# gsneha26/SegAlign

Measured on AMD Instinct MI355X. Metric: Gbp query seeded+filtered+extended per sec, higher is better.
Workload: dtype int32

## Files before the change

segalign_amd/csrc/extend.hip:

```cpp
#include <atomic>
#include <cstdlib>

#include "kernels.h"
#include "kmer_dev.h"

namespace sa {

constexpr int EXT_THREADS = 256;
constexpr int NEG = -(1 << 26);
constexpr int DEAD = -(1 << 29);
constexpr uint64_t TERM_ALL = 0x4040404040404040ull;
constexpr uint32_t BIAS = SEQ_PAD;

__device__ __forceinline__ int f64_to_i32(double x) { return (int)x; }

enum : int { PH_RIGHT = 0, PH_LEFT = 1, PH_FIN = 2, PH_IDLE = 3 };

template <int CTRL, int ROW_MASK = 0xf, int BANK_MASK = 0xf>
__device__ __forceinline__ int dpp_mov(int old, int v) {
    return __builtin_amdgcn_update_dpp(old, v, CTRL, ROW_MASK, BANK_MASK, false);
}
__device__ __forceinline__ uint32_t wave_inclusive_sum(uint32_t v) {
    v += (uint32_t)dpp_mov<0x111>(0, (int)v);
    v += (uint32_t)dpp_mov<0x112>(0, (int)v);
// ... 557 lines not shown
                        }
                        const uint32_t rp = (td >> (4 * j)) & 15u;
                        const uint32_t addr = (rp << 2) | qaddr;
                        const s16x2 e = __builtin_bit_cast(s16x2, *reinterpret_cast<const uint32_t*>(reinterpret_cast<const char*>(s_pk) + addr));
                        const s16x2 Tb = T.yy;
                        T = __builtin_elementwise_add_sat(Tb, e);
                        M = __builtin_elementwise_max(M, T);
                    }
                    m = max((int)M.x, (int)M.y);
                    alive = (m - (int)T.y) <= xdrop;
                }
            }
            walked += 64;
            if (!alive) {
                if (!left) {
                    bestR = m;
                    if (SRC == SRC_CAND && left_known) {
                        best = left_best;
                        phase = PH_FIN;
                    } else {
                        phase = PH_LEFT;
                        walked = 0;
                        T = (s16x2){0, 0};
                        M = (s16x2){0, 0};
                    }
                } else {
                    best = m;
                    phase = PH_FIN;
                }
            } else if (walked + (uint32_t)(64 - CTX_R_BASES) >= long_cap) {
                forward = true;
                phase = PH_FIN;
            }
        }

        const unsigned long long fin = __ballot(phase == PH_FIN);
        const unsigned long long live = __ballot(phase < PH_FIN);
        if (fin != 0ull && (__popcll(fin) >= fin_batch || live == 0ull)) {
            bool cand = false;
            if (phase == PH_FIN && has_hit) cand = forward || bound_passes(a, bestR + best);
            {
                CandRec cr;
                cr.ref_loc = ref_loc; cr.query_loc = query_loc; cr.hidx = hidx;
                stage_append(stage, n_stage, cand, cr, a.cand_list, a.cand_count, a.cand_cap_recs, lane, lane_lt);
            }
            if (a.audit_list) {
                uint2 ar;
                ar.x = ref_loc; ar.y = query_loc;
                wave_append(phase == PH_FIN && has_hit && !cand, ar, a.audit_list, a.audit_count, a.audit_cap, lane, lane_lt);
            }
            unsigned long long need = fin;
            bool got = false;
            Hit mine = {0u, 0u};
            uint32_t mine_idx = 0, mine_known = 0, mine_tm = 0, mine_flags = 3;
            while (need != 0ull) {
                const int avail = buf_cnt - consumed;
                if (avail <= 0) {
                    if (nxt_cnt == 0) break;
                    buf = nxt;
                    buf_idx = nxt_idx;
                    buf_known = nxt_known; buf_tm = nxt_tm; buf_flags = nxt_flags;
                    buf_cnt = nxt_cnt;
                    cur_buf = nxt_buf;
                    consumed = 0;
                    nxt_buf += G;
                    nxt_cnt = buf_count(nxt_buf);
                    nxt = fetch(nxt_buf, nxt_cnt);
                    nxt_idx = f_idx;
                    nxt_known = f_known; nxt_tm = f_tm; nxt_flags = f_flags;
                    continue;
                }
                const int rank = __popcll(need & lane_lt);
                const bool take = ((need >> lane) & 1ull) && rank < avail;
                const int src = (consumed + rank) & 63;
                const uint32_t hr = (uint32_t)__shfl((int)buf.ref_loc, src, 64);
                const uint32_t hq = (uint32_t)__shfl((int)buf.query_loc, src, 64);
                const uint32_t hi = SRC == SRC_CAND ? (uint32_t)__shfl((int)buf_idx, src, 64) : (uint32_t)(cur_buf << 6) + (uint32_t)src;
                uint32_t hk = 0, ht = 0, hf = 3;
                if (SRC == SRC_CAND) {
                    hk = (uint32_t)__shfl((int)buf_known, src, 64);
                    ht = (uint32_t)__shfl((int)buf_tm, src, 64);
                    hf = (uint32_t)__shfl((int)buf_flags, src, 64);
                }
                if (take) {
                    mine.ref_loc = hr;
                    mine.query_loc = hq;
                    mine_idx = hi;
                    mine_known = hk; mine_tm = ht; mine_flags = hf;
                    got = true;
                }
                consumed += min(__popcll(need), avail);
                need &= ~__ballot(take);
            }
            if (phase == PH_FIN) {
                forward = false;
                if (got) {
                    has_hit = true;
                    ref_loc = mine.ref_loc;
                    query_loc = mine.query_loc;
                    hidx = mine_idx;
                    bestR = 0;
                    best = 0;
                    bool skip = false;
                    if (a.rm) skip = !(ref_loc >= a.rm_win_start && ref_loc <= a.rm_win_end);
                    left_known = false;
                    if (skip || ref_loc > a.ref_len || query_loc > a.query_len) {
                        phase = PH_FIN;
                    } else if (SRC == SRC_CAND && mine_flags == 0u) {
                        bestR = (int)mine_known;
                        best = (int)mine_tm;
                        phase = PH_FIN;
                    } else if (SRC == SRC_CAND && mine_flags == 2u) {
                        bestR = (int)mine_known;
                        phase = PH_LEFT;
                        walked = (uint32_t)CTX_L_BASES + a.left_skip;
                        const short t16 = (short)(mine_tm & 0xFFFFu), m16 = (short)(mine_tm >> 16);
                        T = (s16x2){t16, t16};
                        M = (s16x2){m16, m16};
                    } else {
                        phase = PH_RIGHT;
                        walked = 0;
                        T = (s16x2){0, 0};
                        M = (s16x2){0, 0};
                        if (SRC == SRC_CAND && mine_flags == 1u) {
                            left_known = true;
                            left_best = (int)mine_known;
                            if (a.l2_right_state) {
                                walked = (uint32_t)CTX_R_BASES;
                                const short t16 = (short)(mine_tm & 0xFFFFu), m16 = (short)(mine_tm >> 16);
                                T = (s16x2){t16, t16};
                                M = (s16x2){m16, m16};
                            }
                        }
                    }
                } else {
                    has_hit = false;
                    phase = PH_IDLE;
                }
            }
        }
        if (__ballot(phase != PH_IDLE) == 0ull) break;
    }
    stage_flush(stage, n_stage, a.cand_list, a.cand_count, a.cand_cap_recs, lane);
}

constexpr int CTX_THREADS = 1024;
constexpr int CTX_THREADS_MAX = 1024;
constexpr int CTX_STAGE_FLUSH = 32;
constexpr int CTX_STAGE_CAP = CTX_STAGE_FLUSH - 1 + 64 + 1;
constexpr int CLS_TAB = 4096;
constexpr int CLS_TAIL = 256;
constexpr int CLS_LDS_DWORDS = CLS_TAB + CLS_TAIL;
constexpr bool CLS_TRACK_DROP = true;

__device__ __forceinline__ void cls_table_init(uint32_t* __restrict__ s_cls, const int* cls, int nthreads) {
    const int c0 = cls[0], c1 = cls[1], c2 = cls[2], c3 = cls[3];
    for (int i = threadIdx.x; i < CLS_TAB + CLS_TAIL; i += nthreads) {
        const int nb = i < CLS_TAB ? 6 : 4;
        const int f = i < CLS_TAB ? i : i - CLS_TAB;
        int sum = 0, mx = 0;
        for (int k = 0; k < nb; k++) {
            const int x = (f >> (2 * k)) & 3;
            sum += x == 0 ? c0 : x == 1 ? c1 : x == 2 ? c2 : c3;
            mx = max(mx, sum);
        }
        s_cls[i] = ((uint32_t)sum << 16) | ((uint32_t)(sum - mx) & 0xFFFFu);
    }
}

template <int O>
__device__ __forceinline__ uint32_t cls_field_addr(uint32_t w0, uint32_t w1) {
    constexpr uint32_t MASK = 0x3FFCu;
    if (O + 12 <= 32) return O >= 2 ? ((w0 >> (O - 2)) & MASK) : ((w0 << (2 - O)) & MASK);
    return __builtin_amdgcn_alignbit(w1, w0, (uint32_t)(O - 2)) & MASK;
}

__device__ __forceinline__ uint32_t mul24(uint32_t x, uint32_t s_uniform) {
    uint32_t r;
    asm("v_mul_u32_u24 %0, %1, %2" : "=v"(r) : "s"(s_uniform), "v"(x));
    return r;
}

__device__ __forceinline__ void cls_step(const uint32_t* __restrict__ s_tab, uint32_t addr, uint32_t& P, uint32_t& W) {
    const uint32_t e = *reinterpret_cast<const uint32_t*>(reinterpret_cast<const char*>(s_tab) + addr);
    asm("v_pk_add_i16 %0, %1, %2 op_sel:[0,1] op_sel_hi:[1,1]" : "=v"(P) : "v"(P), "v"(e));
    asm("v_min_i16_sdwa %0, %0, %1 dst_sel:WORD_0 dst_unused:UNUSED_PRESERVE src0_sel:WORD_0 src1_sel:WORD_0" : "+v"(P) : "v"(e));
    if (CLS_TRACK_DROP) {
        typedef short s16x2 __attribute__((ext_vector_type(2)));
        W = __builtin_bit_cast(uint32_t, __builtin_elementwise_min(__builtin_bit_cast(s16x2, W), __builtin_bit_cast(s16x2, P)));
    }
}

__device__ __forceinline__ uint32_t cls_seed_state(const ExtendArgs& a) {
    const int cmax = max(max(a.cls[0], a.cls[1]), max(a.cls[2], a.cls[3]));
    return (uint32_t)((int)a.left_skip * max(cmax, 0)) << 16;
}

template <bool ONE_COPY>
__global__ __launch_bounds__(CTX_THREADS_MAX, 8) void extend_filter_cls_kernel(ExtendArgs a) {
    __shared__ __attribute__((aligned(16))) uint32_t s_cls[CLS_LDS_DWORDS];
    extern __shared__ L2Rec s_l2_dyn[];
    cls_table_init(s_cls, a.cls, (int)blockDim.x);
    __syncthreads();
    const uint32_t* __restrict__ s_tail = s_cls + CLS_TAB;
    L2Rec* stage = s_l2_dyn + (threadIdx.x >> 6) * CTX_STAGE_CAP;
    int n_stage = 0;
    const int lane = threadIdx.x & 63;
    const unsigned long long lane_lt = (1ull << lane) - 1ull;
    const int xdrop = a.xdrop;
    const uint4* __restrict__ ctx = reinterpret_cast<const uint4*>(a.td_ctx);
    const uint32_t seed_state = cls_seed_state(a);

    const uint64_t num_buf = (a.num_hits + 63) >> 6;
    const uint64_t n_chunks = (a.num_hits + TD_CHUNK_HITS - 1) / TD_CHUNK_HITS;
    const uint64_t W = (uint64_t)gridDim.x * (blockDim.x >> 6);
    const uint64_t wid = (uint64_t)__builtin_amdgcn_readfirstlane((int)(blockIdx.x * (blockDim.x >> 6) + (threadIdx.x >> 6)));
    const uint64_t c_lo = (wid * n_chunks) / W, c_hi = ((wid + 1) * n_chunks) / W;
    const uint64_t b_lo = c_lo * (TD_CHUNK_HITS / 64);
    const uint64_t b_hi = min(c_hi * (TD_CHUNK_HITS / 64), num_buf);
    if (b_lo >= b_hi) return;
    const uint32_t my_sub = (uint32_t)wid & (uint32_t)(L2_NSUB - 1);
    L2Rec* __restrict__ my_list = a.l2_list + (size_t)my_sub * a.l2_cap;
    uint32_t* __restrict__ my_count = a.l2_count + my_sub * L2_CNT_STRIDE;
    typedef const uint64_t __attribute__((address_space(4))) * HeadPtr;
    HeadPtr head = (HeadPtr)a.td_bits;
    const uint32_t stride16 = (uint32_t)(a.q2_stride >> 4) & 0xFFFFFFu;
    uint32_t cbefore;
    auto locate = [&](uint64_t B) -> uint32_t {
        const uint64_t Bs = B >> 1;
        const uint32_t idx = __builtin_amdgcn_mbcnt_hi((uint32_t)(Bs >> 32), __builtin_amdgcn_mbcnt_lo((uint32_t)Bs, cbefore - 1u + (uint32_t)(B & 1ull)));
        cbefore += (uint32_t)__builtin_popcountll(B);
        return idx;
    };
    struct Stage {
        uint4 c0, tl;
        uint32_t q[7];
        uint32_t query_loc;
    };
    auto merge_q = [&](Stage& S, uint32_t qr0, uint32_t qr1, uint32_t qr2, uint32_t qr3, uint32_t ql0, uint32_t ql1, uint32_t ql2, uint32_t ql3) {
        S.q[0] = qr0; S.q[1] = qr1; S.q[2] = qr2;
        S.q[3] = (qr3 & 0xFFFu) | (ql0 << 12);
        S.q[4] = __builtin_amdgcn_alignbit(ql1, ql0, 20);
        S.q[5] = __builtin_amdgcn_alignbit(ql2, ql1, 20);
        S.q[6] = __builtin_amdgcn_alignbit(ql3, ql2, 20);
    };
    uint64_t w0, w1, w2;
    TdRec hnext;
    auto advance_map = [&](uint64_t b_req) {
        hnext = a.td_rec[locate(w0)];
        w0 = w1;
        w1 = w2;
        w2 = head[b_req + 4];
    };
    auto request = [&](uint64_t b, Stage& S) {
        const uint64_t entry = hnext.off + (uint64_t)((uint32_t)(b << 6) + (uint32_t)lane - hnext.prefix);
        S.c0 = ctx[2 * entry];
        S.tl = ctx[2 * entry + 1];
        const uint32_t query_loc = hnext.qpos + a.seed_size;
        S.query_loc = query_loc;
        const uint32_t lp = a.query_len - query_loc + a.left_skip;
        if (ONE_COPY) {
            uint4 t;
            uint32_t t4;
            const uint8_t* rpp = a.q2_own + ((query_loc >> 4) << 2);
            __builtin_memcpy(&t, __builtin_assume_aligned(rpp, 4), 16);
            __builtin_memcpy(&t4, __builtin_assume_aligned(rpp + 16, 4), 4);
            const uint32_t sr = (query_loc & 15u) << 1;
            uint4 u;
            uint32_t u4;
            const uint8_t* lpp = a.q2_other + ((lp >> 4) << 2);
            __builtin_memcpy(&u, __builtin_assume_aligned(lpp, 4), 16);
            __builtin_memcpy(&u4, __builtin_assume_aligned(lpp + 16, 4), 4);
            const uint32_t sl = (lp & 15u) << 1;
            merge_q(S, __builtin_amdgcn_alignbit(t.y, t.x, sr), __builtin_amdgcn_alignbit(t.z, t.y, sr), __builtin_amdgcn_alignbit(t.w, t.z, sr),
                    __builtin_amdgcn_alignbit(t4, t.w, sr), __builtin_amdgcn_alignbit(u.y, u.x, sl), __builtin_amdgcn_alignbit(u.z, u.y, sl),
                    __builtin_amdgcn_alignbit(u.w, u.z, sl), __builtin_amdgcn_alignbit(u4, u.w, sl));
        } else {
            const uint32_t po = (mul24(query_loc & 15u, stride16) << 4) + ((query_loc >> 4) << 2);
            uint4 t, u;
            __builtin_memcpy(&t, __builtin_assume_aligned(a.q2_own + po, 4), 16);
            const uint32_t qo = (mul24(lp & 15u, stride16) << 4) + ((lp >> 4) << 2);
            __builtin_memcpy(&u, __builtin_assume_aligned(a.q2_other + qo, 4), 16);
            merge_q(S, t.x, t.y, t.z, t.w, u.x, u.y, u.z, u.w);
        }
    };
    auto score = [&](uint64_t b, const Stage& S) {
        const bool valid = (b << 6) + (uint64_t)lane < a.num_hits;
        const uint32_t query_loc = S.query_loc;
        const uint32_t ref_loc = S.c0.x + a.seed_size;
        bool skip = !valid;
        if (a.rm) skip = skip || !(ref_loc >= a.rm_win_start && ref_loc <= a.rm_win_end);
        const uint32_t x0 = S.c0.y ^ S.q[0], x1 = S.c0.z ^ S.q[1], x2 = S.c0.w ^ S.q[2], x3 = S.tl.x ^ S.q[3], x4 = S.tl.y ^ S.q[4],
                       x5 = S.tl.z ^ S.q[5], x6 = S.tl.w ^ S.q[6];
        uint32_t P = 0, Wd = 0;
        cls_step(s_cls, cls_field_addr<0>(x0, x1), P, Wd);
        cls_step(s_cls, cls_field_addr<12>(x0, x1), P, Wd);
        cls_step(s_cls, cls_field_addr<24>(x0, x1), P, Wd);
        cls_step(s_cls, cls_field_addr<4>(x1, x2), P, Wd);
        cls_step(s_cls, cls_field_addr<16>(x1, x2), P, Wd);
        cls_step(s_cls, cls_field_addr<28>(x1, x2), P, Wd);
        cls_step(s_cls, cls_field_addr<8>(x2, x3), P, Wd);
        cls_step(s_cls, cls_field_addr<20>(x2, x3), P, Wd);
        cls_step(s_cls, cls_field_addr<0>(x3, x4), P, Wd);
        const bool r_alive = (int)(short)((CLS_TRACK_DROP ? Wd : P) & 0xFFFFu) >= -xdrop;
        const int bestR = ((int)P >> 16) - (int)(short)(P & 0xFFFFu);
        const uint32_t PR = P;
        P = seed_state; Wd = 0;
        cls_step(s_cls, cls_field_addr<12>(x3, x4), P, Wd);
        cls_step(s_cls, cls_field_addr<24>(x3, x4), P, Wd);
        cls_step(s_cls, cls_field_addr<4>(x4, x5), P, Wd);
        cls_step(s_cls, cls_field_addr<16>(x4, x5), P, Wd);
        cls_step(s_cls, cls_field_addr<28>(x4, x5), P, Wd);
        cls_step(s_cls, cls_field_addr<8>(x5, x6), P, Wd);
        cls_step(s_cls, cls_field_addr<20>(x5, x6), P, Wd);
        cls_step(s_cls, cls_field_addr<0>(x6, 0u), P, Wd);
        cls_step(s_cls, cls_field_addr<12>(x6, 0u), P, Wd);
        cls_step(s_tail, (x6 >> 22) & 0x3FCu, P, Wd);
        const bool l_alive = (int)(short)((CLS_TRACK_DROP ? Wd : P) & 0xFFFFu) >= -xdrop;
        const int bestL = ((int)P >> 16) - (int)(short)(P & 0xFFFFu);
        const bool fwd = !skip && (r_alive || l_alive || bound_passes(a, bestR + bestL));
        const unsigned long long fm = __ballot(fwd);
        if (fm) {
            L2Rec cr;
            cr.ref_loc = ref_loc;
            cr.query_loc = query_loc;
            cr.hidx = (uint32_t)(b << 6) + (uint32_t)lane;
            const uint32_t fl = (r_alive ? 1u : 0u) | (l_alive ? 2u : 0u);
            const uint32_t Ps = (fl == 1u && a.l2_right_state) ? PR : P;
            cr.state = (Ps & 0xFFFF0000u) | ((0u - Ps) & 0xFFFFu);
            cr.meta = (uint32_t)(r_alive ? bestL : bestR) | ((fl ? fl : 3u) << 16);
            const uint32_t rank = __builtin_amdgcn_mbcnt_hi((uint32_t)(fm >> 32), __builtin_amdgcn_mbcnt_lo((uint32_t)fm, 0u));
            if (fwd) stage[n_stage + (int)rank] = cr;
            n_stage += __popcll(fm);
            __builtin_amdgcn_wave_barrier();
            if (n_stage >= CTX_STAGE_FLUSH) {
                const int k = n_stage < 64 ? n_stage : 64;
                stage_flush(stage, k, my_list, my_count, a.l2_cap, lane);
                const int rest = n_stage - k;
                L2Rec tmp = cr;
                if (lane < rest) tmp = stage[k + lane];
                __builtin_amdgcn_wave_barrier();
                if (lane < rest) stage[lane] = tmp;
                __builtin_amdgcn_wave_barrier();
                n_stage = rest;
            }
        }
        if (a.audit_list) {
            uint2 ar;
            ar.x = ref_loc;
            ar.y = query_loc;
            wave_append(valid && !skip && !fwd, ar, a.audit_list, a.audit_count, a.audit_cap, lane, lane_lt);
        }
    };
    Stage SA, SB;
    {
        const uint64_t h0 = head[b_lo];
        w0 = head[b_lo + 1];
        w1 = head[b_lo + 2];
        w2 = head[b_lo + 3];
        cbefore = a.td_chunk[c_lo] + 1u - (uint32_t)(h0 & 1ull);
        hnext = a.td_rec[locate(h0)];
        request(b_lo, SA);
        advance_map(b_lo);
    }
    for (uint64_t b = b_lo; b < b_hi; b += 2) {
        request(b + 1, SB);
        advance_map(b + 1);
        score(b, SA);
        if (b + 1 >= b_hi) break;
        request(b + 2, SA);
        advance_map(b + 2);
        score(b + 1, SB);
    }
    stage_flush(stage, n_stage, my_list, my_count, a.l2_cap, lane);
}

__device__ __forceinline__ int rfl(int v) { return __builtin_amdgcn_readfirstlane(v); }

template <bool COUNT_EXAMINED, bool XDROP_NONNEG>
__device__ __forceinline__ void wave_extend_exact(const ExtendArgs& a, const int* __restrict__ s_tab,
                                                  const uint8_t* __restrict__ R8b, const uint8_t* __restrict__ Qb, int lane,
                                                  uint32_t ref_loc, uint32_t query_loc, int& bestR, int& bposR, int& bestL,
                                                  int& boffL, unsigned long long& examined) {
    const int xdrop = a.xdrop;
    bestR = 0; bposR = -1; bestL = 0; boffL = 0;
    bool skip = false;
    if (a.rm) skip = !(ref_loc >= a.rm_win_start && ref_loc <= a.rm_win_end);
    if (skip) bposR = 0;
    for (int side = skip ? 2 : 0; side < 2; side++) {
        const bool left = side == 1;
        const uint32_t lim = left ? min(ref_loc, query_loc)
                                  : ((ref_loc < a.ref_len && query_loc < a.query_len)
                                         ? min(a.ref_len - ref_loc, a.query_len - query_loc) : 0u);
        uint32_t k0 = left ? 1u : 0u;
        int score_in = 0, best_in = 0, bpos_in = left ? 0 : -1;
        for (;;) {
            const uint32_t k = k0 + 8u * (uint32_t)lane;
            const int64_t rem64 = left ? (int64_t)lim - (int64_t)k + 1 : (int64_t)lim - (int64_t)k;
            const int remaining = rem64 > 8 ? 8 : (rem64 < 0 ? 0 : (int)rem64);
            uint64_t x = 0;
            if (remaining > 0) {
                const uint32_t roff = left ? ref_loc + BIAS - k - 7u : ref_loc + BIAS + k;
                const uint32_t qoff = left ? query_loc + BIAS - k - 7u : query_loc + BIAS + k;
                x = load8u(R8b + roff) | load8u(Qb + qoff);
                if (left) x = __builtin_bswap64(x);
            }
            if (remaining < 8) x |= (remaining <= 0) ? TERM_ALL : (TERM_ALL << (8 * remaining));
            uint32_t run = 0;
            int mx = INT32_MIN, amx = 0;
            {
                const uint32_t xlo = (uint32_t)x, xhi = (uint32_t)(x >> 32);
#pragma unroll
                for (int j = 0; j < 8; j++) {
                    const uint32_t w = j < 4 ? xlo : xhi;
                    run += (uint32_t)s_tab[(w >> (8 * (j & 3))) & 0xffu];
                    const bool up = (int)run > mx;
                    amx = up ? j : amx;
                    mx = up ? (int)run : mx;
                }
            }
            const uint32_t inc = wave_inclusive_sum(run);
            const int base = (int)((uint32_t)score_in + inc - run);
            int mv = (int)((uint32_t)base + (uint32_t)mx), mp = (int)(k + (uint32_t)amx);
            wave_inclusive_max(mv, mp);
            int ev = dpp_mov<0x138>(INT32_MIN, mv);
            int ep = dpp_mov<0x138>(0, mp);
            if (best_in >= ev) { ev = best_in; ep = bpos_in; }
            int score = base, best = ev, bpos = ep;
            uint32_t ex_step = 0;
            chunk8_exact<COUNT_EXAMINED, XDROP_NONNEG>(s_tab, x, k, xdrop, score, best, bpos, ex_step);
            const unsigned long long dm = __ballot(score < (DEAD >> 1));
            if (dm) {
                const int f = __ffsll((long long)dm) - 1;
                best_in = __builtin_amdgcn_readlane(best, f);
                bpos_in = __builtin_amdgcn_readlane(bpos, f);
                if (COUNT_EXAMINED && lane <= f) examined += ex_step;
                break;
            }
            if (COUNT_EXAMINED) examined += ex_step;
            score_in = __builtin_amdgcn_readlane(score, 63);
            best_in = __builtin_amdgcn_readlane(best, 63);
            bpos_in = __builtin_amdgcn_readlane(bpos, 63);
            k0 += 512u;
        }
        if (!left) { bestR = best_in; bposR = bpos_in; }
        else { bestL = best_in; boffL = bpos_in; }
    }
}

struct ExactStage {
    HspRec* st_out;
    EntRec* st_ent;
    int n_out, n_ent;
};

__device__ __forceinline__ void wave_finalize(const ExtendArgs& a, ExactStage& st, int lane, uint32_t ref_loc, uint32_t query_loc,
                                              uint32_t seg, int bestR, int bposR, int bestL, int boffL) {
    const int total = bestR + bestL, extent = bposR + boffL;
    const int cls = classify(a, total);
    if (!cls) return;
    if (cls == 1) {
        if (lane == 0) st.st_out[st.n_out] = make_rec(a, ref_loc, query_loc, boffL, extent, total, seg);
        st.n_out++;
        __builtin_amdgcn_wave_barrier();
        if (st.n_out == 64) { stage_flush(st.st_out, 64, a.out, a.out_count, a.out_cap, lane); st.n_out = 0; __builtin_amdgcn_wave_barrier(); }
    } else {
        if (lane == 0) {
            EntRec er;
            er.ref_loc = ref_loc; er.query_loc = query_loc; er.bposR = bposR; er.boffL = boffL; er.total = total; er.seg = seg;
            st.st_ent[st.n_ent] = er;
        }
        st.n_ent++;
        __builtin_amdgcn_wave_barrier();
        if (st.n_ent == 64) { stage_flush(st.st_ent, 64, a.ent_list, a.ent_count, a.ent_cap_recs, lane); st.n_ent = 0; __builtin_amdgcn_wave_barrier(); }
    }
}

#define EXACT_KERNEL_PROLOGUE()                                                                            \
    __shared__ int s_tab[128];                                                                             \
    __shared__ HspRec s_out[EXT_THREADS / 64][64];                                                         \
    __shared__ EntRec s_ent[EXT_THREADS / 64][64];                                                         \
    if (threadIdx.x < 128) s_tab[threadIdx.x] = threadIdx.x < 64 ? a.sub_mat[threadIdx.x] : NEG;           \
    __syncthreads();                                                                                       \
    ExactStage st = {s_out[threadIdx.x >> 6], s_ent[threadIdx.x >> 6], 0, 0};                             \
    const int lane = threadIdx.x & 63;                                                                     \
    const uint8_t* __restrict__ R8b = a.ref8 - BIAS;                                                       \
    const uint8_t* __restrict__ Qb = a.query - BIAS;                                                       \
    const uint32_t n_cand = min(*a.cand_count, a.cand_cap_recs);                                           \
    const uint32_t G = gridDim.x * (EXT_THREADS / 64);                                                     \
    SEG_TABLE()                                                                                            \
    unsigned long long examined = 0;

#define EXACT_KERNEL_EPILOGUE()                                                                            \
    stage_flush(st.st_out, st.n_out, a.out, a.out_count, a.out_cap, lane);                                 \
    stage_flush(st.st_ent, st.n_ent, a.ent_list, a.ent_count, a.ent_cap_recs, lane);                       \
    if (COUNT_EXAMINED) {                                                                                  \
        unsigned long long v = examined;                                                                   \
        for (int off = 32; off > 0; off >>= 1) v += __shfl_down(v, off, 64);                               \
        if (lane == 0 && v) atomicAdd(a.examined, v);                                                      \
    }

template <bool COUNT_EXAMINED, bool XDROP_NONNEG>
__global__ __launch_bounds__(EXT_THREADS) void extend_exact_kernel(ExtendArgs a) {
    EXACT_KERNEL_PROLOGUE()
    if (a.chain_cap && n_cand <= a.chain_cap) return;
    for (uint32_t i = blockIdx.x * (EXT_THREADS / 64) + (threadIdx.x >> 6); i < n_cand; i += G) {
        const CandRec cr = a.cand_list[i];
        const uint32_t ref_loc = (uint32_t)rfl((int)cr.ref_loc), query_loc = (uint32_t)rfl((int)cr.query_loc);
        const uint32_t hidx = (uint32_t)rfl((int)cr.hidx);
        int bestR, bposR, bestL, boffL;
        wave_extend_exact<COUNT_EXAMINED, XDROP_NONNEG>(a, s_tab, R8b, Qb, lane, ref_loc, query_loc, bestR, bposR, bestL, boffL, examined);
        wave_finalize(a, st, lane, ref_loc, query_loc, seg_of(a, s_seg, hidx), bestR, bposR, bestL, boffL);
    }
    EXACT_KERNEL_EPILOGUE()
}

constexpr uint32_t CHAIN_GAP_MAX = 256;
constexpr uint32_t CHAIN_WALK_EXTRA = 96;

constexpr uint32_t CHAIN_BUCKETS_MIN = 16384, CHAIN_BUCKETS_MAX = 262144;
constexpr uint32_t CHAIN_SORT_MAX = 4096;

constexpr uint32_t CHAIN_QSHIFT = 9;
__device__ __forceinline__ uint32_t chain_bucket_of(uint32_t buckets, uint32_t seg, const CandRec& c) {
    const uint32_t diag = c.ref_loc - c.query_loc;
    return (((diag * 2654435761u) ^ ((c.query_loc >> CHAIN_QSHIFT) * 0x85EBCA6Bu) ^ (seg * 0x9E3779B1u)) >> 14) & (buckets - 1u);
// ... 208 lines not shown
                const uint32_t ke = kb + ((hi - lo + 3u) & ~3u);
#pragma unroll 2
                for (uint32_t t = kb; t < ke; t += 4) {
                    const uint4 kk = *reinterpret_cast<const uint4*>(s_key + t);
                    rank += (kk.x < k ? 1u : 0u) + (kk.y < k ? 1u : 0u) + (kk.z < k ? 1u : 0u) + (kk.w < k ? 1u : 0u);
                }
                s_perm[lo + rank] = (uint16_t)i;
            }
            __syncthreads();
        } else if (threadIdx.x == 0 && a.chain_big) {
            atomicAdd(a.chain_big, 1u);
        }
        const uint32_t rounds = (m_all + blockDim.x - 1) / blockDim.x;
        for (uint32_t r = 0; r < rounds; r++) {
            const uint32_t p = r * blockDim.x + threadIdx.x;
            bool head = false;
            if (p < m_all) {
                const CandRec c = big ? a.chain_tmp[g0 + p] : s_rec[s_perm[p]];
                a.chain_sorted[g0 + p] = c;
                head = true;
                if (!big) {
                    uint32_t lo, hi, kb;
                    bucket_of(p, lo, hi, kb);
                    if (p > lo && !a.chain_no_link) head = chain_is_run_head<XDROP_NONNEG>(a, s_seg, s_tab, R8b, Qb, c, s_rec[s_perm[p - 1]]);
                }
                a.chain_is_head[g0 + p] = head ? 1u : 0u;
            }
            const unsigned long long m = __ballot(head);
            if (m) {
                const int leader = __ffsll((long long)m) - 1;
                uint32_t wbase = 0;
                if (lane == leader) wbase = atomicAdd(a.chain_head_count, (uint32_t)__popcll(m));
                wbase = (uint32_t)__builtin_amdgcn_readlane((int)wbase, leader);
                if (head) a.chain_heads[wbase + (uint32_t)__popcll(m & lane_lt)] = g0 + p;
            }
        }
        __syncthreads();
        ja = jb;
    }
    }
}

template <bool XDROP_NONNEG>
__global__ __launch_bounds__(EXT_THREADS) void extend_exact_chain_kernel(ExtendArgs a) {
    constexpr bool COUNT_EXAMINED = false;
    EXACT_KERNEL_PROLOGUE()
    uint32_t first_cand, n_chain;
    if (!chain_range(a, first_cand, n_chain)) return;
    const uint32_t n_heads = *a.chain_head_count;
    for (uint32_t j = blockIdx.x * (EXT_THREADS / 64) + (threadIdx.x >> 6); j < n_heads; j += G) {
        uint32_t cur = (uint32_t)rfl((int)a.chain_heads[j]);
        for (;;) {
            const CandRec cr = a.chain_sorted[cur];
            const uint32_t ref_loc = (uint32_t)rfl((int)cr.ref_loc), query_loc = (uint32_t)rfl((int)cr.query_loc);
            const uint32_t hidx = (uint32_t)rfl((int)cr.hidx);
            int bestR, bposR, bestL, boffL;
            wave_extend_exact<false, XDROP_NONNEG>(a, s_tab, R8b, Qb, lane, ref_loc, query_loc, bestR, bposR, bestL, boffL, examined);
            wave_finalize(a, st, lane, ref_loc, query_loc, seg_of(a, s_seg, hidx), bestR, bposR, bestL, boffL);
            const int64_t right_end = (int64_t)ref_loc + (int64_t)bposR;
            uint32_t nxt = 0xFFFFFFFFu;
            for (uint32_t m0 = cur + 1; m0 < n_chain; m0 += 64) {
                const uint32_t m = m0 + (uint32_t)lane;
                bool stop_run = false, beyond = false;
                if (m < n_chain) {
                    stop_run = a.chain_is_head[m] != 0u;
                    beyond = (int64_t)a.chain_sorted[m].ref_loc > right_end;
                } else {
                    stop_run = true;
                }
                const unsigned long long sm = __ballot(stop_run), bm = __ballot(beyond);
                const int fs = sm ? __ffsll((long long)sm) - 1 : 64, fb = bm ? __ffsll((long long)bm) - 1 : 64;
                if (fb < fs) { nxt = m0 + (uint32_t)fb; break; }
                if (fs < 64) break;
            }
            if (nxt == 0xFFFFFFFFu) break;
            cur = nxt;
        }
    }
    EXACT_KERNEL_EPILOGUE()
}

__global__ __launch_bounds__(EXT_THREADS) void extend_entropy_kernel(ExtendArgs a) {
    const int lane = threadIdx.x & 63;
    const unsigned long long lane_lt = (1ull << lane) - 1ull;
    const uint8_t* __restrict__ R8 = a.ref8;
    const uint8_t* __restrict__ Q = a.query;
    const uint32_t n = min(*a.ent_count, a.ent_cap_recs);
    const uint32_t stride = gridDim.x * EXT_THREADS;
    const uint32_t rounds = (n + stride - 1) / stride;
    for (uint32_t r = 0; r < rounds; r++) {
        const uint32_t i = r * stride + blockIdx.x * EXT_THREADS + threadIdx.x;
        bool pass = false;
        HspRec rec;
        rec.ref_start = rec.query_start = rec.len = rec.seg = 0; rec.score = 0;
        if (i < n) {
            const EntRec e = a.ent_list[i];
            const int extent = e.bposR + e.boffL;
            int c0 = 0, c1 = 0, c2 = 0, c3 = 0;
            for (int d = -e.boffL; d <= e.bposR; d++) {
                const uint32_t rr = (uint32_t)R8[(int64_t)e.ref_loc + d] >> 3, qq = Q[(int64_t)e.query_loc + d];
                if (rr == qq) { c0 += (rr == 0); c1 += (rr == 1); c2 += (rr == 2); c3 += (rr == 3); }
            }
            const short s0 = (short)c0, s1 = (short)c1, s2 = (short)c2, s3 = (short)c3;
            double entropy = 1.0;
            if ((s0 + s1 + s2 + s3) >= 20) {
                const double len1 = (double)(extent + 1);
                double h = 0.0;
                h += ((double)s0) / len1 * ((s0 != 0) ? log(((double)s0) / len1) : 0.0);
                h += ((double)s1) / len1 * ((s1 != 0) ? log(((double)s1) / len1) : 0.0);
                h += ((double)s2) / len1 * ((s2 != 0) ? log(((double)s2) / len1) : 0.0);
                h += ((double)s3) / len1 * ((s3 != 0) ? log(((double)s3) / len1) : 0.0);
                entropy = -h / (a.log4_double ? 1.3862943611198906 : (double)1.38629436492919921875f);
                for (int u = 0; u < a.entropy_ulps; u++) entropy = nextafter(entropy, 2.0);
                for (int u = 0; u > a.entropy_ulps; u--) entropy = nextafter(entropy, -1.0);
            }
            pass = f64_to_i32(((double)(float)e.total) * entropy) >= a.hspthresh;
            int sc = 0;
            if (entropy > 0) sc = f64_to_i32((double)e.total * entropy);
            rec = make_rec(a, e.ref_loc, e.query_loc, e.boffL, extent, sc, e.seg);
        }
        wave_append(pass, rec, a.out, a.out_count, a.out_cap, lane, lane_lt);
    }
}

void launch_extend_filter(const ExtendArgs& a, hipStream_t s) {
    if (a.num_hits == 0) return;
    const uint64_t num_buf = (a.num_hits + 63) / 64;
    uint64_t waves = num_buf / (uint64_t)(a.bufs_per_wave > 0 ? a.bufs_per_wave : 8);
    const uint64_t max_waves = a.max_waves ? a.max_waves : 4096u;
    if (waves > max_waves) waves = max_waves;
    if (waves < 4) waves = 4;
    const uint32_t blocks = (uint32_t)((waves + 3) / 4);
    if (!a.examined && a.fast_filter == 3) {
        const uint32_t pblocks = (uint32_t)((waves + PK_THREADS / 64 - 1) / (PK_THREADS / 64));
        if (a.src_cand) {
            hipLaunchKernelGGL(extend_filter_packed_kernel<SRC_CAND>, dim3(a.l2_blocks ? a.l2_blocks : 256), dim3(PK_THREADS), 0, s, a);
        } else if (a.td) hipLaunchKernelGGL(extend_filter_packed_kernel<SRC_TD>, dim3(pblocks), dim3(PK_THREADS), 0, s, a);
        else hipLaunchKernelGGL(extend_filter_packed_kernel<SRC_HITS>, dim3(pblocks), dim3(PK_THREADS), 0, s, a);
        return;
    }
    if (a.examined) hipLaunchKernelGGL((extend_filter_kernel<true, false>), dim3(blocks), dim3(EXT_THREADS), 0, s, a);
    else if (a.fast_filter) hipLaunchKernelGGL((extend_filter_kernel<false, true>), dim3(blocks), dim3(EXT_THREADS), 0, s, a);
    else hipLaunchKernelGGL((extend_filter_kernel<false, false>), dim3(blocks), dim3(EXT_THREADS), 0, s, a);
}

void launch_extend_filter_cls(const ExtendArgs& a, hipStream_t s) {
    if (a.num_hits == 0) return;
    uint64_t waves = (a.num_hits + TD_CHUNK_HITS - 1) / TD_CHUNK_HITS;
    if (a.ctx_waves && waves > a.ctx_waves) waves = a.ctx_waves;
    uint32_t threads = a.ctx_threads ? a.ctx_threads : (uint32_t)CTX_THREADS;
    threads = std::min<uint32_t>(CTX_THREADS_MAX, std::max<uint32_t>(64, threads & ~63u));
    const uint32_t wpb = threads / 64;
    const uint32_t blocks = (uint32_t)((waves + wpb - 1) / wpb);
    const size_t lds = wpb * CTX_STAGE_CAP * sizeof(L2Rec);
    const bool one_copy = a.cls_one_copy != 2;
    if (one_copy) hipLaunchKernelGGL(extend_filter_cls_kernel<true>, dim3(blocks), dim3(threads), lds, s, a);
    else hipLaunchKernelGGL(extend_filter_cls_kernel<false>, dim3(blocks), dim3(threads), lds, s, a);
}

void launch_chain_group(const ExtendArgs& a, hipStream_t s) {
    if (a.num_hits == 0 || !a.chain_cap) return;
    hipLaunchKernelGGL(chain_count_kernel, dim3(1024), dim3(256), 0, s, a);
    hipLaunchKernelGGL(chain_scan_kernel, dim3(CHAIN_BUCKETS_MAX / CHAIN_SCAN_TILE), dim3(CHAIN_SCAN_THREADS), 0, s, a);
    hipLaunchKernelGGL(chain_scatter_kernel, dim3(1024), dim3(256), 0, s, a);
    const size_t sort_lds = (size_t)a.chain_group_max * (sizeof(uint32_t) + sizeof(CandRec) + sizeof(uint16_t)) + 4 * CHAIN_SORT_GROUP * sizeof(uint32_t);
    static std::atomic<size_t> sort_lds_set[64];
    int dev = 0;
    (void)hipGetDevice(&dev);
    if (sort_lds > 48 * 1024 && dev >= 0 && dev < 64 && sort_lds_set[dev].load(std::memory_order_acquire) < sort_lds) {
        (void)hipFuncSetAttribute(reinterpret_cast<const void*>(&chain_sort_link_kernel<true>), hipFuncAttributeMaxDynamicSharedMemorySize, (int)sort_lds);
        size_t seen = sort_lds_set[dev].load(std::memory_order_relaxed);
        while (seen < sort_lds && !sort_lds_set[dev].compare_exchange_weak(seen, sort_lds, std::memory_order_release)) {}
    }
    hipLaunchKernelGGL((chain_sort_link_kernel<true>), dim3(a.chain_sort_blocks ? a.chain_sort_blocks : 4096), dim3(a.chain_sort_threads ? a.chain_sort_threads : 256),
                       sort_lds, s, a);
}
uint32_t chain_num_buckets() { return CHAIN_BUCKETS_MAX; }
void launch_extend_exact_chain(const ExtendArgs& a, hipStream_t s) {
    if (a.num_hits == 0 || !a.chain_cap) return;
    hipLaunchKernelGGL((extend_exact_chain_kernel<true>), dim3(a.long_blocks), dim3(EXT_THREADS), 0, s, a);
}

void launch_extend_exact(const ExtendArgs& a, hipStream_t s) {
    if (a.num_hits == 0) return;
    const bool nonneg = a.xdrop >= 0;
    if (a.examined) {
        if (nonneg) hipLaunchKernelGGL((extend_exact_kernel<true, true>), dim3(a.long_blocks), dim3(EXT_THREADS), 0, s, a);
        else hipLaunchKernelGGL((extend_exact_kernel<true, false>), dim3(a.long_blocks), dim3(EXT_THREADS), 0, s, a);
    } else {
        if (nonneg) hipLaunchKernelGGL((extend_exact_kernel<false, true>), dim3(a.long_blocks), dim3(EXT_THREADS), 0, s, a);
        else hipLaunchKernelGGL((extend_exact_kernel<false, false>), dim3(a.long_blocks), dim3(EXT_THREADS), 0, s, a);
    }
}

void launch_extend_entropy(const ExtendArgs& a, hipStream_t s) {
    if (a.num_hits == 0) return;
    hipLaunchKernelGGL(extend_entropy_kernel, dim3(a.ent_blocks), dim3(EXT_THREADS), 0, s, a);
}

}
```

Baseline: 1.234.

## Stage per-wave td_rec and query windows in LDS for cls extend kernel

In the one-copy cls filter kernel, each wave now loads a 64-entry tile of td_rec records and a 64-dword window of the packed query (own and other strands) into LDS, refilling only when a lane falls outside the window. Per-hit record and query reads then come from LDS instead of scattered global loads. The main loop is also restructured so the odd tail is scored after the loop, and the host raises the dynamic LDS limit. This adds LDS footprint per block, which may reduce occupancy, and adds ballot checks plus refill paths on every request.

Result: faster. 1.275, median of 6 (+3.3%).

```diff
diff --git a/segalign_amd/csrc/extend.hip b/segalign_amd/csrc/extend.hip
--- a/segalign_amd/csrc/extend.hip
+++ b/segalign_amd/csrc/extend.hip
@@ -733,6 +733,10 @@
 constexpr int CLS_TAIL = 256;
 constexpr int CLS_LDS_DWORDS = CLS_TAB + CLS_TAIL;
 constexpr bool CLS_TRACK_DROP = true;
+constexpr int CLS_TILE = 64;
+constexpr int CLS_WIN_DWORDS = 5;
+constexpr uint32_t CLS_WIN_SPAN = CLS_TILE - CLS_WIN_DWORDS;
+constexpr int CLS_TILE_BYTES = CLS_TILE * (int)sizeof(TdRec) + 2 * CLS_TILE * 4;
 
 __device__ __forceinline__ void cls_table_init(uint32_t* __restrict__ s_cls, const int* cls, int nthreads) {
     const int c0 = cls[0], c1 = cls[1], c2 = cls[2], c3 = cls[3];
@@ -780,14 +784,13 @@
 template <bool ONE_COPY>
 __global__ __launch_bounds__(CTX_THREADS_MAX, 8) void extend_filter_cls_kernel(ExtendArgs a) {
     __shared__ __attribute__((aligned(16))) uint32_t s_cls[CLS_LDS_DWORDS];
-    extern __shared__ L2Rec s_l2_dyn[];
+    extern __shared__ __attribute__((aligned(16))) L2Rec s_l2_dyn[];
     cls_table_init(s_cls, a.cls, (int)blockDim.x);
     __syncthreads();
     const uint32_t* __restrict__ s_tail = s_cls + CLS_TAB;
     L2Rec* stage = s_l2_dyn + (threadIdx.x >> 6) * CTX_STAGE_CAP;
     int n_stage = 0;
     const int lane = threadIdx.x & 63;
-    const unsigned long long lane_lt = (1ull << lane) - 1ull;
     const int xdrop = a.xdrop;
     const uint4* __restrict__ ctx = reinterpret_cast<const uint4*>(a.td_ctx);
     const uint32_t seed_state = cls_seed_state(a);
@@ -826,14 +829,62 @@
         S.q[6] = __builtin_amdgcn_alignbit(ql3, ql2, 20);
     };
     uint64_t w0, w1, w2;
+    uint64_t wc = 0;
     TdRec hnext;
+    typedef uint32_t u32x4 __attribute__((ext_vector_type(4)));
+    typedef u32x4 __attribute__((address_space(3))) * LdsU4;
+    typedef uint32_t __attribute__((address_space(3))) * LdsU32;
+    LdsU4 s_td = nullptr;
+    LdsU32 s_qr = nullptr, s_ql = nullptr;
+    uint32_t td0 = 0, dr0 = 0, dl0 = 0;
+    const uint32_t q2_last = (uint32_t)(a.q2_stride >> 2) - 1u;
+    if (ONE_COPY) {
+        char* tiles = reinterpret_cast<char*>(s_l2_dyn) + (size_t)(blockDim.x >> 6) * (CTX_STAGE_CAP * sizeof(L2Rec)) + (size_t)(threadIdx.x >> 6) * CLS_TILE_BYTES;
+        s_td = (LdsU4)tiles;
+        s_qr = (LdsU32)(tiles + CLS_TILE * sizeof(TdRec));
+        s_ql = s_qr + CLS_TILE;
+    }
+    auto rare_lane = [&]() -> uint32_t {
+        uint32_t l = (uint32_t)lane;
+        asm volatile("" : "+v"(l));
+        return l;
+    };
+    auto tile_td = [&](uint32_t base) {
+        const uint32_t l = rare_lane();
+        const TdRec r = a.td_rec[min(base + l, a.td_m)];
+        __builtin_amdgcn_wave_barrier();
+        s_td[l] = u32x4{r.prefix, r.qpos, (uint32_t)r.off, (uint32_t)(r.off >> 32)};
+        __builtin_amdgcn_wave_barrier();
+        td0 = base;
+    };
+    auto tile_q = [&](uint32_t own_dword, uint32_t other_dword) {
+        const uint32_t nr = own_dword, nl = other_dword > CLS_WIN_SPAN ? other_dword - CLS_WIN_SPAN : 0u;
+        const uint32_t l = rare_lane();
+        const uint32_t vr = reinterpret_cast<const uint32_t*>(a.q2_own)[min(nr + l, q2_last)];
+        const uint32_t vl = reinterpret_cast<const uint32_t*>(a.q2_other)[min(nl + l, q2_last)];
+        __builtin_amdgcn_wave_barrier();
+        s_qr[l] = vr;
+        s_ql[l] = vl;
+        __builtin_amdgcn_wave_barrier();
+        dr0 = nr;
+        dl0 = nl;
+    };
     auto advance_map = [&](uint64_t b_req) {
-        hnext = a.td_rec[locate(w0)];
+        if (ONE_COPY) wc = w0;
+        else hnext = a.td_rec[locate(w0)];
         w0 = w1;
         w1 = w2;
         w2 = head[b_req + 4];
     };
     auto request = [&](uint64_t b, Stage& S) {
+        if (ONE_COPY) {
+            const uint32_t idx = locate(wc);
+            if (__builtin_expect(__ballot(idx - td0 >= (uint32_t)CLS_TILE) != 0ull, 0)) tile_td((uint32_t)__builtin_amdgcn_readfirstlane((int)idx));
+            const u32x4 r = s_td[idx - td0];
+            hnext.prefix = r.x;
+            hnext.qpos = r.y;
+            hnext.off = (uint64_t)r.z | ((uint64_t)r.w << 32);
+        }
         const uint64_t entry = hnext.off + (uint64_t)((uint32_t)(b << 6) + (uint32_t)lane - hnext.prefix);
         S.c0 = ctx[2 * entry];
         S.tl = ctx[2 * entry + 1];
@@ -841,18 +892,30 @@
         S.query_loc = query_loc;
         const uint32_t lp = a.query_len - query_loc + a.left_skip;
         if (ONE_COPY) {
-            uint4 t;
-            uint32_t t4;
-            const uint8_t* rpp = a.q2_own + ((query_loc >> 4) << 2);
-            __builtin_memcpy(&t, __builtin_assume_aligned(rpp, 4), 16);
-            __builtin_memcpy(&t4, __builtin_assume_aligned(rpp + 16, 4), 4);
-            const uint32_t sr = (query_loc & 15u) << 1;
-            uint4 u;
-            uint32_t u4;
-            const uint8_t* lpp = a.q2_other + ((lp >> 4) << 2);
-            __builtin_memcpy(&u, __builtin_assume_aligned(lpp, 4), 16);
-            __builtin_memcpy(&u4, __builtin_assume_aligned(lpp + 16, 4), 4);
-            const uint32_t sl = (lp & 15u) << 1;
+            uint4 t, u;
+            uint32_t t4, u4;
+            const uint32_t dr = query_loc >> 4, dl = lp >> 4;
+            const uint32_t sr = (query_loc & 15u) << 1, sl = (lp & 15u) << 1;
+            bool tiled = true;
+            if (__builtin_expect(__ballot(dr - dr0 > CLS_WIN_SPAN || dl - dl0 > CLS_WIN_SPAN) != 0ull, 0)) {
+                tile_q((uint32_t)__builtin_amdgcn_readfirstlane((int)dr), (uint32_t)__builtin_amdgcn_readfirstlane((int)dl));
+                tiled = __ballot(dr - dr0 > CLS_WIN_SPAN || dl - dl0 > CLS_WIN_SPAN) == 0ull;
+            }
+            if (tiled) {
+                const LdsU32 rp = s_qr + (dr - dr0), lq = s_ql + (dl - dl0);
+                t = make_uint4(rp[0], rp[1], rp[2], rp[3]);
+                t4 = rp[4];
+                u = make_uint4(lq[0], lq[1], lq[2], lq[3]);
+                u4 = lq[4];
+            } else {
+                const uint8_t* rpp = a.q2_own + (dr << 2);
+                __builtin_memcpy(&t, __builtin_assume_aligned(rpp, 4), 16);
+                __builtin_memcpy(&t4, __builtin_assume_aligned(rpp + 16, 4), 4);
+                const uint8_t* lpp = a.q2_other + (dl << 2);
+                __builtin_memcpy(&u, __builtin_assume_aligned(lpp, 4), 16);
+                __builtin_memcpy(&u4, __builtin_assume_aligned(lpp + 16, 4), 4);
+                __builtin_amdgcn_s_waitcnt(0x0F70);
+            }
             merge_q(S, __builtin_amdgcn_alignbit(t.y, t.x, sr), __builtin_amdgcn_alignbit(t.z, t.y, sr), __builtin_amdgcn_alignbit(t.w, t.z, sr),
                     __builtin_amdgcn_alignbit(t4, t.w, sr), __builtin_amdgcn_alignbit(u.y, u.x, sl), __builtin_amdgcn_alignbit(u.z, u.y, sl),
                     __builtin_amdgcn_alignbit(u.w, u.z, sl), __builtin_amdgcn_alignbit(u4, u.w, sl));
@@ -930,7 +993,7 @@
             uint2 ar;
             ar.x = ref_loc;
             ar.y = query_loc;
-            wave_append(valid && !skip && !fwd, ar, a.audit_list, a.audit_count, a.audit_cap, lane, lane_lt);
+            wave_append(valid && !skip && !fwd, ar, a.audit_list, a.audit_count, a.audit_cap, lane, (1ull << rare_lane()) - 1ull);
         }
     };
     Stage SA, SB;
@@ -940,19 +1003,28 @@
         w1 = head[b_lo + 2];
         w2 = head[b_lo + 3];
         cbefore = a.td_chunk[c_lo] + 1u - (uint32_t)(h0 & 1ull);
-        hnext = a.td_rec[locate(h0)];
+        if (ONE_COPY) {
+            const uint32_t i0 = a.td_chunk[c_lo];
+            const uint32_t ql0 = a.td_rec[i0].qpos + a.seed_size;
+            wc = h0;
+            tile_td(i0);
+            tile_q(ql0 >> 4, (a.query_len - ql0 + a.left_skip) >> 4);
+        } else {
+            hnext = a.td_rec[locate(h0)];
+        }
         request(b_lo, SA);
         advance_map(b_lo);
     }
-    for (uint64_t b = b_lo; b < b_hi; b += 2) {
+    uint64_t b = b_lo;
+    for (; b + 1 < b_hi; b += 2) {
         request(b + 1, SB);
         advance_map(b + 1);
         score(b, SA);
-        if (b + 1 >= b_hi) break;
         request(b + 2, SA);
         advance_map(b + 2);
         score(b + 1, SB);
     }
+    if (b < b_hi) score(b, SA);
     stage_flush(stage, n_stage, my_list, my_count, a.l2_cap, lane);
 }
 
@@ -1467,8 +1539,16 @@
     threads = std::min<uint32_t>(CTX_THREADS_MAX, std::max<uint32_t>(64, threads & ~63u));
     const uint32_t wpb = threads / 64;
     const uint32_t blocks = (uint32_t)((waves + wpb - 1) / wpb);
-    const size_t lds = wpb * CTX_STAGE_CAP * sizeof(L2Rec);
     const bool one_copy = a.cls_one_copy != 2;
+    const size_t lds = wpb * (CTX_STAGE_CAP * sizeof(L2Rec) + (one_copy ? (size_t)CLS_TILE_BYTES : 0));
+    static std::atomic<size_t> cls_lds_set[64];
+    int dev = 0;
+    (void)hipGetDevice(&dev);
+    if (one_copy && lds > 32 * 1024 && dev >= 0 && dev < 64 && cls_lds_set[dev].load(std::memory_order_acquire) < lds) {
+        (void)hipFuncSetAttribute(reinterpret_cast<const void*>(&extend_filter_cls_kernel<true>), hipFuncAttributeMaxDynamicSharedMemorySize, (int)lds);
+        size_t seen = cls_lds_set[dev].load(std::memory_order_relaxed);
+        while (seen < lds && !cls_lds_set[dev].compare_exchange_weak(seen, lds, std::memory_order_release)) {}
+    }
     if (one_copy) hipLaunchKernelGGL(extend_filter_cls_kernel<true>, dim3(blocks), dim3(threads), lds, s, a);
     else hipLaunchKernelGGL(extend_filter_cls_kernel<false>, dim3(blocks), dim3(threads), lds, s, a);
 }
```
